# tomneda/DABstar

Hardware: AMD Instinct MI355X
Metric: DAB Mode-I ensembles/s (2.048 MS/s IQ->MSC bytes) per GPU; FIB CRC match % (higher is better)
Workload: dtype f32+i32

## Files before the change

### dabstar_amd/csrc/engine.cpp

```cpp
#include "engine.h"
#include "viterbi_core.h"
#include "fig00.h"
#include <algorithm>
#include <cstddef>
#include <cstring>
#include <map>
#include <string>
#include <tuple>
#include <vector>

int dabx_engine::build_msc_classes()
{
  const EngineDev &d = dev;
  have_fast = false;
  fast = MscFast{};
  for (void *q : fast_allocs) {
    (void)hipFree(q);
    allocs.erase(std::remove(allocs.begin(), allocs.end(), q), allocs.end());
  }
  fast_allocs.clear();
  for (auto &sc : subch_host) sc.fast_class = 0;
  if (d.max_subch <= 0) return 0;
  struct Key { int kbps, prot, shortf, cu; bool operator<(const Key &o) const { return std::tie(kbps, prot, shortf, cu) < std::tie(o.kbps, o.prot, o.shortf, o.cu); } };
  std::map<Key, std::vector<uint32_t>> groups;
// ... 674 lines not shown

int dabx_process(dabx_engine *e, int max_frames, int sync)
{
  if (!e || max_frames < 0) return DABX_E_ARG;
  if (int rc = use_device(e)) return rc;
  if (e->classes_dirty) {
    if (int rc = e->build_msc_classes()) return rc;
    e->classes_dirty = false;
  }
  if (e->dl.open && max_frames > 0) {
    const int need = (e->pending_frames + max_frames + MSC_BATCH_FRAMES - 1) / MSC_BATCH_FRAMES;
    int free_slots = 0;
    {
      std::lock_guard<std::mutex> lk(e->dl.mu);
      for (const auto &sl : e->dl.slots) free_slots += sl.state == Delivery::FREE;
    }
    if (free_slots < need) {
      set_error("dabx_process: the call closes %d chunks, %d host slabs are free (dabx_delivery_next / dabx_delivery_release)", need, free_slots);
      return DABX_E_STATE;
    }
  }
  const bool some_locked = !e->locked_host || 2 * __atomic_load_n(e->locked_host, __ATOMIC_RELAXED) >= e->dev.n_streams;
  const bool async_acquire = !e->cfg.dc_iq_correction && e->cir.n_corr == 0 && e->spectrum.n_on == 0 && (e->cfg.acquire_mode == 2 || (e->cfg.acquire_mode == 0 && some_locked));
  for (int i = 0; i < max_frames; i++) {
    if (e->ss.prep_pending && e->pending_frames >= 4) {
      DABX_HIP(hipStreamWaitEvent(e->stream, e->ss.prep_b_done, 0));
      e->ss.prep_pending = false;
    }
    const bool all_locked = e->locked_host && __atomic_load_n(e->locked_host, __ATOMIC_RELAXED) == e->dev.n_streams;
    const int cir_cap = e->cir.n_on > 0 ? cir_step_cap(e, false) : 0;
    int rc = launch_front_step(e->dev, e->ss, e->mk, async_acquire, all_locked, e->scope.n_on > 0 ? &e->scope.dev : nullptr,
                               e->cir.n_on > 0 ? &e->cir.dev : nullptr, cir_cap, e->spectrum.n_on > 0 ? &e->spectrum.dev : nullptr);
    if (rc) return rc;
    if (cir_cap > 0) cir_step_cap(e, true);
    if (e->cir.n_on > 0 && (cir_cap > 0 || e->cir.n_corr > 0)) e->cir.launches++;
    if (e->scope.n_on > 0) e->scope.launches++;
    if (e->spectrum.n_on > 0) e->spectrum.launches++;
    if (e->tiis.n_on > 0) {
      if ((rc = launch_tii(e->dev, e->tiis.dev, e->stream))) return rc;
      e->tiis.launches++;
    }
    if ((rc = fig_step(e))) return rc;
    e->level_dirty = true;
    if (++e->pending_frames == MSC_BATCH_FRAMES || i == max_frames - 1) {
      DeliverDev dv{};
      int dl_slot = -1, dl_dev = -1;
      if (e->dl.open && (rc = e->delivery_begin(&dv, &dl_slot, &dl_dev))) return rc;
      e->dev.snap = e->snap_buf[e->ss.batch_parity];
      hipStream_t tail = e->stream;
      const bool with_eti = e->dl.open && e->dl.eti();
      const EtiDev eti = with_eti ? e->dl.eti_dev(dl_dev) : EtiDev{};
      rc = launch_msc_batch(e->dev, 4 * e->pending_frames, e->have_fast ? &e->fast : nullptr, e->ss, e->mk, e->dl.open ? &dv : nullptr, &tail,
                            e->pkt.dev.n > 0 ? &e->pkt.dev : nullptr, e->pad.dev.n > 0 ? &e->pad.dev : nullptr, e->mot.dev.n > 0 ? &e->mot.dev : nullptr,
                            e->car.dev.n > 0 ? &e->car.dev : nullptr, with_eti ? &eti : nullptr, e->mpa.dev.n > 0 ? &e->mpa.dev : nullptr, &e->mpa_launches,
                            e->aac.dev.n > 0 ? &e->aac.dev : nullptr, &e->aac_launches);
      if (rc) {
// ... 412 lines not shown
```

### dabstar_amd/csrc/pipeline.h

```cpp
#pragma once
#include "dabx_internal.h"
#include "ring_fmt.h"
#include <cstddef>

namespace dabx {

#ifndef DABX_MSC_BATCH
#define DABX_MSC_BATCH 7
#endif
constexpr int MSC_SLOTS = DABX_MSC_BATCH > 7 ? 64 : 32;
constexpr int MSC_BATCH_FRAMES = DABX_MSC_BATCH;
constexpr int SF_SLOTS = 16;
constexpr int ACQ_NEED = 20 * TU + 50 + (TF + 1) + (TN + 50 + 21) + 64;
constexpr int FRAME_NEED = TF + 2 * TU;
constexpr int FEW_STREAMS = 48;

enum StreamState : int32_t { ST_INIT = 0, ST_WAIT_SYNC = 1, ST_EVAL_SYNC = 2 };

struct StreamCtl {
  unsigned long long rd;
  unsigned long long sym0_pos;
  long long cif_no;
  long long msc_done_cif;
  long long frames;
// ... 282 lines not shown
  const SubchDev &sc = e.subch[(size_t)q.s * e.max_subch + q.j];
  q.r = b.msc_done + q.k;
  const long long valid_from = sc.start_cif + 16;
  q.valid = sc.active && q.r < b.cif_no && q.r >= valid_from;
  q.out_idx = sc.cif_out + (q.r - (b.msc_done > valid_from ? b.msc_done : valid_from));
  return q;
}
__device__ __forceinline__ size_t tdi_off(long long cif, int i)
{
  return (size_t)(cif & (TDI_SLOTS - 1)) * CIF_BITS + (size_t)(i & 15) * (CIF_BITS / 16) + (size_t)(i >> 4);
}
#endif

struct PacketDev;
struct PadDev;
struct MotDev;
struct CarouselDev;
struct Mp2AudioDev;
struct AacStreamDev;
struct ScopeDev;
struct CirDev;
struct SpecDev;
extern const char *const kStepKernelNames[N_STEP_KERNELS];
int launch_front_step(const EngineDev &e, EngineStreams &ss, Marker &mk, bool async_acquire, bool all_locked, const ScopeDev *scope = nullptr,
                      const CirDev *cir = nullptr, int cir_cap = 0, const SpecDev *spec = nullptr);
int launch_msc_batch(const EngineDev &e, int cifs, const MscFast *fast, EngineStreams &ss, Marker &mk, const DeliverDev *dv = nullptr,
                     hipStream_t *tail = nullptr, const PacketDev *pk = nullptr, const PadDev *pad = nullptr, const MotDev *mot = nullptr,
                     const CarouselDev *car = nullptr, const EtiDev *eti = nullptr, const Mp2AudioDev *mp2a = nullptr, long long *mp2a_launches = nullptr,
                     const AacStreamDev *aac = nullptr, long long *aac_launches = nullptr);
int launch_dciq(const EngineDev &e, int mode, hipStream_t st);
int launch_level_exact(const EngineDev &e, hipStream_t st);
int launch_commit(const EngineDev &e, int stream, unsigned long long n, hipStream_t st);
int launch_fic_only(const EngineDev &e, hipStream_t st, int first, int count);
int launch_i16_to_sym(const int16_t *soft, uint8_t *sym, size_t n, hipStream_t st);
int launch_stage_msc_block(const EngineDev &e, const int16_t *soft_dev, int blk, bool closes_cif, hipStream_t st);
int launch_msc_inject(const EngineDev &e, int stream, const int16_t *soft_dev, int n_cifs, int first, hipStream_t st);
int launch_msc_advance(const EngineDev &e, const int32_t *counts_dev, hipStream_t st);
int launch_fic_inject(const EngineDev &e, int stream, const int16_t *soft_dev, hipStream_t st);
int launch_fic_decode(const EngineDev &e, const int32_t *present_dev, hipStream_t st);
int launch_demap_inject(const EngineDev &e, int parity, int stream, const float2 *spec_dev, const float2 *null_dev, float clock_err, int np_sel, hipStream_t st);
int launch_demap_frame(const EngineDev &e, unsigned step_count, const int32_t *present_dev, int schedule, hipStream_t st, const ScopeDev *scope = nullptr);
int launch_msc_prep(const EngineDev &e, int cifs, const MscLaunch &L, hipStream_t st, Marker &mk);
int launch_msc_vitT(const EngineDev &e, int cifs, const MscLaunch &L, hipStream_t st, Marker &mk);
int launch_deliver_front(const EngineDev &e, const DeliverDev &dv, hipStream_t st);
int launch_deliver_msc(const EngineDev &e, const DeliverDev &dv, hipStream_t st, bool with_lf);
int launch_deliver_lf(const EngineDev &e, const DeliverDev &dv, hipStream_t st);
int launch_deliver_dg(const EngineDev &e, const DeliverDev &dv, const PacketDev &pk, hipStream_t st);
int launch_deliver_pad(const EngineDev &e, const DeliverDev &dv, const PadDev &pd, hipStream_t st);
// ... 19 lines not shown
```

### dabstar_amd/csrc/pipeline.hip

```cpp
#include <type_traits>
#include "pipeline.h"
#include "packet_core.h"
#include "pad_core.h"
#include "mot_core.h"
#include "carousel_core.h"
#include "mp2_core.h"
#include "aac_core.h"
#include <algorithm>
#include "ofdm_core.h"
#include "scope_core.h"
#include "cir_core.h"
#include "spectrum_core.h"
#include "viterbi_core.h"
#include "fec_core.h"
#include "acq_walk.h"
#include "level_par.h"
#include "fig00.h"

namespace dabx {

__device__ __forceinline__ void front_prio() { __builtin_amdgcn_s_setprio(3); }

template <class T> __device__ __forceinline__ T uniform_load(const T *p)
{
// ... 583 lines not shown
    Nco nco;
    nco.init(phase0, f, tid);
    const RingView<RF> rv(ring, e.ring_len, rd);
    float2 v[8];
#pragma unroll
    for (int u = 0; u < 8; u++) { v[u] = nco.mix(rv.at(tid + 256 * u)); nco.step(); }
    const int start = prs_correlate_block(v, c.sync_thr, e.strongest, t, lds, peak, red, tid);
    __syncthreads();
    if (start >= 0) break;
    sync_failed<RF>(e, s, tid, rv, rd, phase0, f, peak, red, true);
    new_state = ST_WAIT_SYNC;
    if (wr - c.rd < (unsigned long long)(ACQ_NEED + FRAME_NEED)) break;
  }
  if (new_state < 0) return;
  if (tid == 0 && e.exact_level) e.level_pos[s] = c.rd;
  if (tid == 0 && e.anchor_level) { c.lvl_anchor_pos = c.lvl_approx_pos = c.rd; c.lvl_anchor_S = c.s_level; }
  if (tid == 0 && new_state == ST_EVAL_SYNC && e.locked_count) __hip_atomic_fetch_add(e.locked_count, 1, __ATOMIC_RELAXED, __HIP_MEMORY_SCOPE_SYSTEM);
  __threadfence();
  __syncthreads();
  if (tid == 0) __hip_atomic_store(&c.state, new_state, __ATOMIC_RELEASE, __HIP_MEMORY_SCOPE_AGENT);
}

template <int RF>
__global__ __launch_bounds__(256, RF == RING_CF32 ? 3 : 4) void k_frame_head(EngineDev e, DevTables t)
{
  front_prio();
  __shared__ float2 lds[FFT_LDS_FLOAT2];
  __shared__ __attribute__((aligned(16))) float peak[TU];
  __shared__ float red[8];
  __shared__ float mag[160];
  __shared__ int s_state;
  const int s = blockIdx.x, tid = threadIdx.x;
  StreamCtl &c = e.ctl[s];
  const typename RingFmt<RF>::Elem *ring = stream_ring<RF>(e, s);
  if (tid < 76) e.sym_off[(size_t)s * 76 + tid] = -1;
  if (tid == 0) {
    c.frame_ok = 0;
    s_state = __hip_atomic_load(&c.state, __ATOMIC_ACQUIRE, __HIP_MEMORY_SCOPE_AGENT);
  }
  __syncthreads();
  if (s_state != ST_EVAL_SYNC) return;
  __builtin_amdgcn_fence(__ATOMIC_ACQUIRE, "agent");
  if (e.wr[s] - c.rd < (unsigned long long)FRAME_NEED) return;
  const unsigned long long rd = c.rd;
  const int phase0 = c.nco_phase;
  const int f = (int)roundf(c.f_bb);
  float2 v[8];
  Nco nco;
  nco.init(phase0, f, tid);
  const RingView<RF> rv(ring, e.ring_len, rd);
  float abs_a = 0.f, abs_b = 0.f;
#pragma unroll
  for (int u = 0; u < 8; u++) { const float2 x = rv.at(tid + 256 * u); abs_a += cabsf_level(x); v[u] = nco.mix(x); nco.step(); }
  const int start = prs_correlate_block(v, c.sync_thr, e.strongest, t, lds, peak, red, tid);
// ... 34 lines not shown
    }
    if (correction != 0) clock_err = 0.0f;
    f_bb = f_sync;
  }
  e.nco_tid[(size_t)s * 256 + tid] = Nco::tid_factor((int)roundf(f_bb), tid);
  if (tid < 75) {
    double2 b, st;
    Nco::block_consts(nco_advance(phase0, f, (long long)start + TU), (int)roundf(f_bb), (long long)tid * TS + TG, b, st);
    e.nco_sym[(size_t)s * 76 + tid] = b;
    if (tid == 0) e.nco_sym[(size_t)s * 76 + 75] = st;
    e.sym_off[(size_t)s * 76 + tid] = (int32_t)((rd + (unsigned long long)start + TU + (unsigned long long)tid * TS) % (unsigned long long)e.ring_len);
  }
  if (tid == 0) {
    c.start_index = start;
    c.head_abs_a = abs_a; c.head_abs_b = abs_b;
    c.sample_count = start + TU;
    c.sym0_pos = rd + start;
    c.phase_sym1 = nco_advance(phase0, f, (long long)start + TU);
    c.correction = correction;
    c.f_sync = f_sync; c.f_bb = f_bb; c.clock_err = clock_err;
    c.f_frame = (int)roundf(f_bb);
    c.frame_ok = 1;
  }
}

__host__ __device__ constexpr int sym_blocks_per_stream(int n_streams) { return n_streams >= FEW_STREAMS ? 15 : (n_streams >= 16 ? 25 : 75); }
template <int RF>
__global__ __launch_bounds__(256, 3) void k_symbols_persistent(EngineDev e, DevTables t)
{
  front_prio();
  __shared__ float2 lds[FFT_LDS_FLOAT2];
  __shared__ float red3[3][4];
  const int s = blockIdx.y + e.s0, tid = threadIdx.x;
  int l = blockIdx.x;
  int off = uniform_load(e.sym_off + (size_t)s * 76 + l);
  double2 nco_base = uniform_load(e.nco_sym + (size_t)s * 76 + l);
  const double2 nco_step = uniform_load(e.nco_sym + (size_t)s * 76 + 75);
  if (off < 0) return;
  typedef RingFmt<RF> Fmt;
  const typename Fmt::Elem *ring = stream_ring<RF>(e, s);
  const unsigned len = (unsigned)e.ring_len;
  const bool two = tid + 256 < TG;
  typename Fmt::Elem nx[12];
  auto request = [&](int o) {
    auto at = [&](unsigned i) { unsigned a = (unsigned)o + i; if (a >= len) a -= len; return ring_elem<RF>(ring, a); };
    if (RF != RING_CF32) {
// ... 460 lines not shown

struct SrcFic {
  const uint8_t *sym;
  const uint16_t *map;
  typedef ushort4 Key;
  struct Raw { uint8_t a, b, c, d; };
  __device__ Key key(int t) const { return *reinterpret_cast<const ushort4 *>(map + 4 * t); }
  __device__ uint8_t ld(uint16_t idx) const { return sym[idx == PUNCT ? 0 : idx]; }
  __device__ Raw raw(Key m) const { return {ld(m.x), ld(m.y), ld(m.z), ld(m.w)}; }
  __device__ static int cv(uint8_t v, uint16_t idx) { return vit_sym_from_u8(idx == PUNCT ? (uint8_t)127 : v); }
  __device__ VitSyms syms(Raw r, Key m) const { return {cv(r.a, m.x), cv(r.b, m.y), cv(r.c, m.z), cv(r.d, m.w)}; }
};

__global__ __launch_bounds__(256) void k_fic_frame(EngineDev e, DevTables t, int first, int count)
{
  front_prio();
  __shared__ __attribute__((aligned(16))) char wtab[4][VIT_BLK * 16];
  __shared__ uint32_t fibw[4][24];
  __shared__ uint32_t raw[4][32];
  __shared__ uint8_t crc_ok[12];
  __shared__ uint32_t encw[4][26];
  __shared__ int ber_err[4];
  __shared__ uint16_t s_crc[256];
  const int s = blockIdx.x, wave = threadIdx.x >> 6, lane = threadIdx.x & 63;
  StreamCtl &c = e.ctl[s];
  if (e.flag_sync && first == 0 && count == 4) seq_wait(e.fic_seq + s, e.step_seq, e.seq_timeouts);
  if (!c.frame_ok) return;
  s_crc[threadIdx.x] = t.crc_ccitt[threadIdx.x];
  const int fic = first + wave;
  if (wave < count) {
    SrcFic src{e.fic_sym + (size_t)s * 3 * K2 + fic * FIC_IN, t.fic_map};
    uint32_t *dec = e.vit_scratch + ((size_t)s * 4 + fic) * (size_t)e.vit_stride;
    const VitLaneConst k = vit_lane_const(lane);
    if (e.tie_mode == 2) vit_forward<2>(src, FIC_OUT + 6, wtab[wave], dec, lane, k);
    else if (e.tie_mode) vit_forward<1>(src, FIC_OUT + 6, wtab[wave], dec, lane, k);
    else vit_forward<0>(src, FIC_OUT + 6, wtab[wave], dec, lane, k);
    __builtin_amdgcn_fence(__ATOMIC_RELEASE, "workgroup");
    __builtin_amdgcn_s_waitcnt(0);
    vit_traceback(dec, FIC_OUT, lane, raw[wave]);
    __builtin_amdgcn_fence(__ATOMIC_RELEASE, "wavefront");
    __builtin_amdgcn_wave_barrier();
    uint32_t dw = 0;
    if (lane < 24) { dw = vit_output_word(raw[wave], lane); fibw[fic][lane] = dw ^ t.prbs_words[lane]; }
    if (lane < 24) encw[wave][lane] = dw;
    if (lane >= 24 && lane < 26) encw[wave][lane] = 0;
    __builtin_amdgcn_fence(__ATOMIC_RELEASE, "wavefront");
    __builtin_amdgcn_wave_barrier();
    {
      const uint8_t *eb = reinterpret_cast<const uint8_t *>(encw[wave]);
      auto dbit = [&](int i) -> unsigned { return i < 0 ? 0u : (unsigned)((eb[i >> 3] >> (7 - (i & 7))) & 1); };
      const int t0 = 13 * lane;
      unsigned sr = 0;
#pragma unroll
      for (int q = 6; q >= 1; q--) sr = (sr << 1) | dbit(t0 - q);
      int err = 0;
      const uint8_t *sym = e.fic_sym + (size_t)s * 3 * K2 + fic * FIC_IN;
      for (int i = t0; i < t0 + 13 && i < FIC_OUT + 6; i++) {
        sr = ((sr << 1) | dbit(i)) & 0xFFu;
        const ushort4 m = *reinterpret_cast<const ushort4 *>(t.fic_map + 4 * i);
        const unsigned p0 = __builtin_popcount(sr & 109u) & 1u, p1 = __builtin_popcount(sr & 79u) & 1u, p2 = __builtin_popcount(sr & 83u) & 1u;
        if (m.x != PUNCT) err += (unsigned)(sym[m.x] > 127) != p0;
        if (m.y != PUNCT) err += (unsigned)(sym[m.y] > 127) != p1;
        if (m.z != PUNCT) err += (unsigned)(sym[m.z] > 127) != p2;
        if (m.w != PUNCT) err += (unsigned)(sym[m.w] > 127) != p0;
      }
      err = wave_sum_int(err);
      if (lane == 0) ber_err[fic] = err;
    }
  }
  __syncthreads();
  const int slot = (int)(c.frames % e.out_frames);
  uint8_t *fo = e.fib_out + ((size_t)s * e.out_frames + slot) * 12 * 32;
  const int fib0 = 3 * first, nfib = 3 * count;
  __shared__ int fib_cif[12];
  if ((int)threadIdx.x < nfib) {
    const int fibi = fib0 + threadIdx.x;
    const uint8_t *b = reinterpret_cast<const uint8_t *>(&fibw[fibi / 3][0]) + (fibi % 3) * 32;
    const uint8_t good = crc16_check_bytes(b, 30, s_crc);
    crc_ok[fibi] = good;
    e.fib_crc[((size_t)s * e.out_frames + slot) * 12 + fibi] = good;
    int cif = -1;
    int hi, lo;
    if (good && fib_fig00_counter(b, &hi, &lo)) cif = hi * 250 + lo;
    fib_cif[fibi] = cif;
  }
  for (int i = threadIdx.x; i < 24 * count; i += 256) reinterpret_cast<uint32_t *>(fo)[24 * first + i] = fibw[first + i / 24][i % 24];
  __syncthreads();
  if (threadIdx.x == 0) {
    int ratio = c.fic_ratio, cif_count = c.cif_count;
    long long ok = 0;
    for (int fibi = fib0; fibi < fib0 + nfib; fibi++) {
      if (crc_ok[fibi]) {
        ok++;
        if (fib_cif[fibi] >= 0) cif_count = fib_cif[fibi];
        if (ratio < 10) ratio++;
      } else if (ratio > 0) ratio--;
    }
    c.fic_ratio = ratio; c.cif_count = cif_count;
    c.fib_ok += ok; c.fib_total += nfib;
    int bits = c.fic_bits, errs = c.fic_errors, blk = c.fic_block;
    for (int f = first; f < first + count; f++) {
      bits += FIC_IN; errs += ber_err[f];
      if (++blk == 40) { c.fic_status_errors = errs; c.fic_status_bits = bits; blk = 0; errs /= 2; bits /= 2; }
    }
    c.fic_bits = bits; c.fic_errors = errs; c.fic_block = blk;
  }
}

template <int RF>
__global__ __launch_bounds__(256) void k_frame_tail(EngineDev e, DevTables t)
{
  front_prio();
  __shared__ float2 lds[FFT_LDS_FLOAT2];
  __shared__ float red[8];
  __shared__ float s_fbb;
  const int s = blockIdx.x, tid = threadIdx.x;
  StreamCtl &c = e.ctl[s];
  if (!c.frame_ok) return;
  const float LNQ = -1.00000500003333e-5f;
  float2 cpp = make_float2(0.f, 0.f);
  float absp = 0.f;
  if (tid < 75) { cpp = e.cp_part[(size_t)s * 75 + tid]; absp = e.abs_part[(size_t)s * 76 + tid]; }
  typedef RingFmt<RF> Fmt;
  const typename Fmt::Elem *ring = stream_ring<RF>(e, s);
  const unsigned long long base = c.sym0_pos + TU + 75ull * TS;
  const RingView<RF> rv(ring, e.ring_len, base);
  typename Fmt::Elem xr[8];
#pragma unroll
  for (int u = 0; u < 8; u++) xr[u] = rv.code(TG + tid + 256 * u);
  constexpr int N_REST = (TN - TU + 255) / 256;
  typename Fmt::Elem xq[N_REST];
#pragma unroll
  for (int k = 0; k < N_REST; k++) {
    const int i = min(tid + 256 * k, TN - TU - 1);
    xq[k] = rv.code(i < TG ? i : i + TU);
  }
  asm volatile("" ::: "memory");
  float cre = cpp.x, cim = cpp.y, sym_w = 0.f;
// ... 65 lines not shown
      auto upd = [&lv](float mean, float qn) { lv += (1.0f - qn) * (mean - lv); };
      const int start = c.start_index;
      upd(c.head_abs_a * (1.0f / (float)TU), __expf((float)TU * LNQ));
      if (start > 0) upd(c.head_abs_b / (float)start, __expf((float)start * LNQ));
      lv = lv * __expf((float)(75 * TS) * LNQ) + (1.0f - __expf((float)TS * LNQ)) * sym_w;
      upd(an * (1.0f / (float)TN), __expf((float)TN * LNQ));
      if (!e.exact_level) c.s_level = lv;
    }
    if (e.frame_pos) {
      const size_t slot = (size_t)s * e.out_frames + (size_t)(c.frames % e.out_frames);
      e.frame_pos[slot] = (long long)c.sym0_pos; e.frame_start[slot] = c.start_index;
    }
    c.sample_count = sample_count;
    c.rd = base + TN;
    c.lvl_approx_pos = c.rd;
    { const int h = (int)(c.frames % LVL_HIST); c.lvl_hist_pos[h] = c.rd; c.lvl_hist_S[h] = c.s_level; }
    c.nco_phase = nco_advance(phase_null, f2, TN);
    c.cif_no += 4;
    c.frames += 1;
    c.np_sel ^= 1;
    c.sync_thr = 2.0f * e.threshold;
    c.state = ST_EVAL_SYNC;
  }
}

template <int RF>
__global__ __launch_bounds__(128) void k_level_exact(EngineDev e)
{
  front_prio();
  const int s = blockIdx.x, tid = threadIdx.x, lane = tid & 63;
  const int wave = __builtin_amdgcn_readfirstlane(tid >> 6);
  StreamCtl &c = e.ctl[s];
  constexpr int CH = 1024;
  __shared__ __attribute__((aligned(16))) float chunk[2][CH + 32];
  const unsigned long long rd0 = e.level_pos[s];
  const unsigned long long rd1 = __hip_atomic_load(&c.rd, __ATOMIC_RELAXED, __HIP_MEMORY_SCOPE_AGENT);
  if (rd1 <= rd0) return;
  const unsigned long long n = rd1 - rd0;
  typedef RingFmt<RF> Fmt;
  const typename Fmt::Elem *ring = stream_ring<RF>(e, s);
  const unsigned len = (unsigned)e.ring_len;
  typename Fmt::Elem raw[CH / 64];
  unsigned raw_ok = 0;
  __shared__ float s_pk;
  auto request = [&](unsigned long long p0) {
    const unsigned o0 = (unsigned)((rd0 + p0) % len);
// ... 445 lines not shown
}

int launch_spectrum_rows_test(const float2 *in, int n, float *state, float *lin, float *db, float *ext, const float *window, hipStream_t st)
{
  const DevTables *t;
  if (int rc = get_tables(&t)) return rc;
  hipLaunchKernelGGL(k_spectrum_rows_test, dim3(1), dim3(256), 0, st, in, n, state, lin, db, ext, window, *t);
  DABX_HIP(hipGetLastError());
  return 0;
}

static int launch_spectrum(const EngineDev &e, const DevTables &t, const SpecDev *sd, hipStream_t st)
{
  if (!sd || sd->n <= 0) return 0;
  DABX_LAUNCH_RING(e, k_spectrum, dim3(sd->n), dim3(256), 0, st, e, t, *sd);
  DABX_HIP(hipGetLastError());
  return 0;
}

const char *const kStepKernelNames[N_STEP_KERNELS] = {"k_acquire", "k_frame_head", "k_symbols", "k_demap_frame", "k_fic_frame", "k_frame_tail",
                                                      "k_msc_prep", "k_msc_vitT", "k_msc_frame", "k_dabplus", "k_demap_fic", "k_packet", "k_pad", "k_mot",
                                                      "k_carousel", "k_eti"};

int launch_front_step(const EngineDev &e_in, EngineStreams &ss, Marker &mk, bool async_acquire, bool all_locked, const ScopeDev *scope, const CirDev *cir, int cir_cap,
                      const SpecDev *spec)
{
  const DevTables *t;
  int rc = get_tables(&t);
  if (rc) return rc;
  EngineDev e = e_in;
  e.parity = (int)(ss.step_count++ & 1u);
  e.step_seq = ss.step_count;
  e.flag_sync = (ss.d && ss.fic_on_d && e.sym_seq) ? 1 : 0;
  hipStream_t st = ss.a;
  if (all_locked && !e.exact_level) {
  } else if (async_acquire && ss.q) {
    const bool go = !ss.acq_in_flight || hipEventQuery(ss.acq_done) == hipSuccess;
    if (go || e.exact_level) {
      if (ss.acq_a_pending) { DABX_HIP(hipStreamWaitEvent(ss.q, ss.acq_a_done, 0)); ss.acq_a_pending = false; }
      if (e.exact_level) {
        if (ss.tail_recorded) DABX_HIP(hipStreamWaitEvent(ss.q, ss.tail_done, 0));
        DABX_LAUNCH_RING(e, k_level_exact, dim3(e.n_streams), dim3(128), 0, ss.q, e);
      }
      if (go) { mk.begin(0, ss.q); DABX_LAUNCH_RING(e, k_acquire, dim3(e.n_streams), dim3(256), 0, ss.q, e, *t, 1); mk.end(0, ss.q); }
      DABX_HIP(hipEventRecord(ss.acq_done, ss.q));
      ss.acq_in_flight = true;
    }
  } else {
    if (ss.acq_in_flight) { DABX_HIP(hipStreamWaitEvent(st, ss.acq_done, 0)); ss.acq_in_flight = false; }
    if (e.exact_level) DABX_LAUNCH_RING(e, k_level_exact, dim3(e.n_streams), dim3(128), 0, st, e);
    mk.begin(0, st); DABX_LAUNCH_RING(e, k_acquire, dim3(e.n_streams), dim3(256), 0, st, e, *t, 1); mk.end(0, st);
    if (ss.q && ss.acq_a_done) { DABX_HIP(hipEventRecord(ss.acq_a_done, st)); ss.acq_a_pending = true; }
  }
  if ((rc = launch_cir(e, *t, cir, cir_cap, st))) return rc;
  if ((rc = launch_cir_corr(e, *t, cir, st))) return rc;
  mk.begin(1, st); DABX_LAUNCH_RING(e, k_frame_head, dim3(e.n_streams), dim3(256), 0, st, e, *t); mk.end(1, st);
  if ((rc = launch_spectrum(e, *t, spec, st))) return rc;
  mk.begin(2, st); DABX_LAUNCH_RING(e, k_symbols_persistent, dim3(sym_blocks_per_stream(e.n_streams), e.n_streams), dim3(256), 0, st, e, *t); mk.end(2, st);
#define DABX_DEMAP_DISPATCH(KERNEL, ...)                                                                                         \
  do {                                                                                                                          \
    const int st_ = e.demap.soft_type == 3 ? 3 : e.demap.soft_type == 2 ? 2 : 1;                                                \
    if (e.demap.track_mer) {                                    \
      if (e.tie_mode) {                                                                                                         \
        if (st_ == 3) hipLaunchKernelGGL((KERNEL<3, true, true>), __VA_ARGS__);                                                 \
        else if (st_ == 2) hipLaunchKernelGGL((KERNEL<2, true, true>), __VA_ARGS__);                                            \
        else hipLaunchKernelGGL((KERNEL<1, true, true>), __VA_ARGS__);                                                          \
      } else {                                                                                                                  \
        if (st_ == 3) hipLaunchKernelGGL((KERNEL<3, false, true>), __VA_ARGS__);                                                \
        else if (st_ == 2) hipLaunchKernelGGL((KERNEL<2, false, true>), __VA_ARGS__);                                           \
        else hipLaunchKernelGGL((KERNEL<1, false, true>), __VA_ARGS__);                                                         \
      }                                                                                                                         \
    } else if (e.tie_mode) {                                                                                                    \
      if (st_ == 3) hipLaunchKernelGGL((KERNEL<3, true, false>), __VA_ARGS__);                                                  \
      else if (st_ == 2) hipLaunchKernelGGL((KERNEL<2, true, false>), __VA_ARGS__);                                             \
      else hipLaunchKernelGGL((KERNEL<1, true, false>), __VA_ARGS__);                                                           \
    } else {                                                                                                                    \
      if (st_ == 3) hipLaunchKernelGGL((KERNEL<3, false, false>), __VA_ARGS__);                                                 \
      else if (st_ == 2) hipLaunchKernelGGL((KERNEL<2, false, false>), __VA_ARGS__);                                            \
      else hipLaunchKernelGGL((KERNEL<1, false, false>), __VA_ARGS__);                                                          \
// ... 5 lines not shown
  if (ss.d && ss.fic_on_d) {
    hipLaunchKernelGGL(k_sym_publish, dim3((e.n_streams + 63) / 64), dim3(64), 0, st, e);
    if ((rc = launch_scope(e, *t, scope, ss.d))) return rc;
    mk.begin(3, ss.d);
    DABX_DEMAP_DISPATCH(k_demap_whole, dim3(e.n_streams), dim3(DEMAP_THREADS), 0, ss.d, e, *t);
    mk.end(3, ss.d);
    ss.demap_in_flight = true; ss.demap_unrecorded = true;
  } else if (ss.d) {
    if (ss.demap_in_flight) { DABX_HIP(hipStreamWaitEvent(st, ss.demap_done, 0)); ss.demap_in_flight = false; }
    if ((rc = launch_scope(e, *t, scope, st))) return rc;
    mk.begin(10, st);
    DABX_DEMAP_DISPATCH(k_demap_fic, dim3(e.n_streams), dim3(DEMAP_THREADS), 0, st, e, *t);
    mk.end(10, st);
    DABX_HIP(hipEventRecord(ss.fic_go, st));
    DABX_HIP(hipStreamWaitEvent(ss.d, ss.fic_go, 0));
    mk.begin(3, ss.d); demap(ss.d, 3, 75); mk.end(3, ss.d);
    DABX_HIP(hipEventRecord(ss.demap_done, ss.d));
    ss.demap_in_flight = true;
  } else {
    if ((rc = launch_scope(e, *t, scope, st))) return rc;
    mk.begin(3, st); demap(st, 0, 75); mk.end(3, st);
  }
  mk.begin(4, st); hipLaunchKernelGGL(k_fic_frame, dim3(e.n_streams), dim3(256), 0, st, e, *t, 0, 4); mk.end(4, st);
  mk.begin(5, st); DABX_LAUNCH_RING(e, k_frame_tail, dim3(e.n_streams), dim3(256), 0, st, e, *t); mk.end(5, st);
  if (e.exact_level && ss.tail_done) { DABX_HIP(hipEventRecord(ss.tail_done, st)); ss.tail_recorded = true; }
  DABX_HIP(hipGetLastError());
  return 0;
}

int launch_msc_batch(const EngineDev &e, int cifs, const MscFast *fast, EngineStreams &ss, Marker &mk, const DeliverDev *dv, hipStream_t *tail,
                     const PacketDev *pk, const PadDev *pad, const MotDev *mot, const CarouselDev *car, const EtiDev *eti, const Mp2AudioDev *mp2a,
                     long long *mp2a_launches, const AacStreamDev *aac, long long *aac_launches)
{
  const DevTables *t;
  int rc = get_tables(&t);
  if (rc) return rc;
  if (tail) *tail = ss.a;
  if (e.fic_only || e.max_subch <= 0 || !e.msc_out) {
    if (dv && (rc = launch_deliver_msc(e, *dv, ss.a, true))) return rc;
    if (dv && eti && (rc = launch_eti_back(e, *eti, ss.a, mk, false))) return rc;
    return 0;
  }
  const int jobs = e.n_streams * cifs * e.max_subch;
  auto wait_for_demapper = [&](hipStream_t who) -> int {
    if (!ss.demap_in_flight) return 0;
    if (ss.demap_unrecorded) { DABX_HIP(hipEventRecord(ss.demap_done, ss.d)); ss.demap_unrecorded = false; }
    DABX_HIP(hipStreamWaitEvent(who, ss.demap_done, 0));
// ... 253 lines not shown
```

### dabstar_amd/csrc/viterbi_core.h

```cpp
#pragma once
#include <hip/hip_runtime.h>
#include <stdint.h>
#include "wave_ops.h"

namespace dabx {

constexpr int VIT_BLK = 60;
constexpr int VIT_DW = 30;

__host__ __device__ inline int vit_words(int nbits) { return (nbits + 6 + VIT_DW - 1) / VIT_DW; }
__host__ __device__ inline int vit_blocks(int nbits) { return (nbits + 6 + VIT_BLK - 1) / VIT_BLK; }
__host__ __device__ inline size_t vit_scratch_words(int nbits) { return (size_t)vit_blocks(nbits) * 2 * 64; }

struct VitSyms { int x0, x1, x2, x3; };

__device__ __forceinline__ int vit_sym_from_i16(int16_t s)
{
  int v = (int16_t)(s + 127);
  v = v < 0 ? 0 : (v > 255 ? 255 : v);
  return 2 * v - 255;
}
__device__ __forceinline__ int vit_sym_from_u8(uint8_t sym) { return 2 * (int)sym - 255; }
__device__ __forceinline__ int vit_sym_from_i16_sat(int16_t s)
{
  int v = (int)s + 127;
// ... 79 lines not shown
__device__ __forceinline__ void vit_step_simd(int &m, unsigned &acc, const char *wrow, const VitLaneConst &k)
{
  constexpr int CEIL = RULE == 1 ? 65535 : 32767;
  const int w = *reinterpret_cast<const int16_t *>(wrow + k.pat[C]);
  const int bm = (w + 1020) >> 1;
  const int partner = vit_exchange<C>(m, k.lane);
  int a = m + bm, b = partner + (1020 - bm);
  a = a > CEIL ? CEIL : a; b = b > CEIL ? CEIL : b;
  const int dd = __mul24(a - b, k.sgn[C]);
  m = a < b ? a : b;
  if constexpr (RULE == 1) asm("v_cmp_le_i32 vcc, 0, %1\n\tv_addc_co_u32 %0, vcc, %0, %0, vcc" : "+v"(acc) : "v"(dd) : "vcc");
  else asm("v_cmp_lt_i32 vcc, 0, %1\n\tv_addc_co_u32 %0, vcc, %0, %0, vcc" : "+v"(acc) : "v"(dd) : "vcc");
}
__device__ __forceinline__ int vit_wave_min(int v) { return wave_min_int(v); }
template <int C, int RULE>
__device__ __forceinline__ void vit_pair_simd(int &m, unsigned &acc, const char *row, const VitLaneConst &k)
{
  vit_step_simd<C, RULE>(m, acc, row, k);
  const int m0_before = __builtin_amdgcn_readfirstlane(m);
  vit_step_simd<C + 1, RULE>(m, acc, row + 16, k);
  if (m0_before > (RULE == 1 ? 60000 : 30000)) m -= vit_wave_min(m);
}

template <int RULE = 0, class Src>
__device__ __forceinline__ void vit_forward(const Src &src, int nsteps, char *wtab, uint32_t *dec, int lane,
                                            const VitLaneConst &k)
{
  int m = RULE ? (lane == 0 ? 0 : 1000) : (lane == 0 ? 0 : 2000);
  const int nblk = (nsteps + VIT_BLK - 1) / VIT_BLK;
  const bool fetcher = lane < VIT_BLK;
  auto tclamp = [&](int t) { return t < nsteps ? t : 0; };
  typename Src::Key k1 = src.key(tclamp(lane));
  typename Src::Raw rw = src.raw(k1);
  VitSyms s = src.syms(rw, k1);
  if (!(fetcher && lane < nsteps)) s = VitSyms{0, 0, 0, 0};
  k1 = src.key(tclamp(VIT_BLK + lane));
  for (int b = 0; b < nblk; b++) {
    const int tn = (b + 1) * VIT_BLK + lane;
    const typename Src::Raw rn = src.raw(k1);
    const typename Src::Key kn = k1;
    k1 = src.key(tclamp(tn + VIT_BLK));
    if (lane < VIT_BLK) {
      const int y0 = s.x0 + s.x3;
      short v[8];
#pragma unroll
      for (int q = 0; q < 8; q++)
        v[q] = (short)(((q & 4) ? -y0 : y0) + ((q & 2) ? -s.x1 : s.x1) + ((q & 1) ? -s.x2 : s.x2));
      int4 pk;
      pk.x = (unsigned short)v[0] | ((unsigned)(unsigned short)v[1] << 16);
      pk.y = (unsigned short)v[2] | ((unsigned)(unsigned short)v[3] << 16);
      pk.z = (unsigned short)v[4] | ((unsigned)(unsigned short)v[5] << 16);
      pk.w = (unsigned short)v[6] | ((unsigned)(unsigned short)v[7] << 16);
      *reinterpret_cast<int4 *>(wtab + lane * 16) = pk;
    }
    __builtin_amdgcn_fence(__ATOMIC_RELEASE, "wavefront");
    __builtin_amdgcn_wave_barrier();
    unsigned acc = 0;
#pragma unroll
    for (int h = 0; h < VIT_BLK / VIT_DW; h++) {
#pragma unroll
      for (int s6 = 0; s6 < VIT_DW; s6 += 6) {
        const char *row = wtab + (h * VIT_DW + s6) * 16;
        if constexpr (RULE != 0) {
          vit_pair_simd<0, RULE>(m, acc, row + 0 * 16, k);
          vit_pair_simd<2, RULE>(m, acc, row + 2 * 16, k);
          vit_pair_simd<4, RULE>(m, acc, row + 4 * 16, k);
        } else {
          vit_step<0>(m, acc, row + 0 * 16, k);
          vit_step<1>(m, acc, row + 1 * 16, k);
          vit_step<2>(m, acc, row + 2 * 16, k);
          vit_step<3>(m, acc, row + 3 * 16, k);
          vit_step<4>(m, acc, row + 4 * 16, k);
          vit_step<5>(m, acc, row + 5 * 16, k);
        }
      }
      dec[(size_t)(b * (VIT_BLK / VIT_DW) + h) * 64 + lane] = RULE == 0 ? acc ^ k.inv30 : acc;
      acc = 0;
    }
    __builtin_amdgcn_wave_barrier();
    s = src.syms(rn, kn);
    if (!(fetcher && tn < nsteps)) s = VitSyms{0, 0, 0, 0};
  }
}

constexpr int VIT_RAW_WORDS = 312;

struct VitMask6 { unsigned long long m5, m4, m3, m2, m1, m0; };
template <int G> __device__ __forceinline__ VitMask6 vit_tb_masks(unsigned hist)
{
  VitMask6 r;
  r.m5 = __builtin_amdgcn_ballot_w64(((hist >> (VIT_DW - 1 - (6 * G + 5))) & 1u) != 0u);
  r.m4 = __builtin_amdgcn_ballot_w64(((hist >> (VIT_DW - 1 - (6 * G + 4))) & 1u) != 0u);
  r.m3 = __builtin_amdgcn_ballot_w64(((hist >> (VIT_DW - 1 - (6 * G + 3))) & 1u) != 0u);
  r.m2 = __builtin_amdgcn_ballot_w64(((hist >> (VIT_DW - 1 - (6 * G + 2))) & 1u) != 0u);
  r.m1 = __builtin_amdgcn_ballot_w64(((hist >> (VIT_DW - 1 - (6 * G + 1))) & 1u) != 0u);
  r.m0 = __builtin_amdgcn_ballot_w64(((hist >> (VIT_DW - 1 - (6 * G + 0))) & 1u) != 0u);
  return r;
}
__device__ __forceinline__ void vit_tb_chain(const VitMask6 &q, int &j, unsigned &acc)
{
  int jc, js;
#define DABX_TB_STEP(M, BIT)                                                                                                    \
  "s_andn2_b32 %[jc], %[j], " #BIT "\n\ts_or_b32 %[js], %[j], " #BIT "\n\ts_bitcmp1_b64 %[" #M "], %[j]\n\t"                        \
  "s_cselect_b32 %[j], %[js], %[jc]\n\t"
  asm volatile(DABX_TB_STEP(m5, 1) DABX_TB_STEP(m4, 2) DABX_TB_STEP(m3, 4) DABX_TB_STEP(m2, 8) DABX_TB_STEP(m1, 16) DABX_TB_STEP(m0, 32)
               "s_brev_b32 %[jc], %[j]\n\ts_lshl_b32 %[acc], %[acc], 6\n\ts_lshr_b32 %[jc], %[jc], 26\n\ts_or_b32 %[acc], %[acc], %[jc]"
               : [jc] "=&s"(jc), [js] "=&s"(js), [acc] "+s"(acc), [j] "+s"(j)
               : [m5] "s"(q.m5), [m4] "s"(q.m4), [m3] "s"(q.m3), [m2] "s"(q.m2), [m1] "s"(q.m1), [m0] "s"(q.m0)
               : "scc");
#undef DABX_TB_STEP
}
template <int NG>
__device__ __forceinline__ VitMask6 vit_tb_word(unsigned hist, unsigned nxt, VitMask6 ahead, int &j, unsigned &acc)
{
  VitMask6 a = ahead;
  if constexpr (NG >= 5) { const VitMask6 b = vit_tb_masks<3>(hist); vit_tb_chain(a, j, acc); a = b; }
  if constexpr (NG >= 4) { const VitMask6 b = vit_tb_masks<2>(hist); vit_tb_chain(a, j, acc); a = b; }
  if constexpr (NG >= 3) { const VitMask6 b = vit_tb_masks<1>(hist); vit_tb_chain(a, j, acc); a = b; }
  if constexpr (NG >= 2) { const VitMask6 b = vit_tb_masks<0>(hist); vit_tb_chain(a, j, acc); a = b; }
  const VitMask6 b = vit_tb_masks<4>(nxt);
  vit_tb_chain(a, j, acc);
  return b;
}

__device__ __forceinline__ void vit_traceback(const uint32_t *dec, int nbits, int lane, uint32_t *raw)
{
  const int nsteps = __builtin_amdgcn_readfirstlane(nbits + 6);
  int j = 0;
  int wi = (nsteps - 1) / VIT_DW;
  unsigned hist = dec[(size_t)wi * 64 + lane];
  VitMask6 ahead;
  {
    const unsigned nxt = wi > 0 ? dec[(size_t)(wi - 1) * 64 + lane] : 0u;
    unsigned acc = 0;
    const int n_top = nsteps - wi * VIT_DW;
    if (n_top % 6 == 0) {
      switch (n_top / 6) {
        case 5: ahead = vit_tb_word<5>(hist, nxt, vit_tb_masks<4>(hist), j, acc); break;
        case 4: ahead = vit_tb_word<4>(hist, nxt, vit_tb_masks<3>(hist), j, acc); break;
        case 3: ahead = vit_tb_word<3>(hist, nxt, vit_tb_masks<2>(hist), j, acc); break;
        case 2: ahead = vit_tb_word<2>(hist, nxt, vit_tb_masks<1>(hist), j, acc); break;
        default: ahead = vit_tb_word<1>(hist, nxt, vit_tb_masks<0>(hist), j, acc); break;
      }
    } else {
      for (int s = n_top - 1; s >= 0; --s) {
        const unsigned hv = (unsigned)__builtin_amdgcn_readlane((int)hist, __builtin_amdgcn_readfirstlane(j));
        const unsigned k = (hv >> (VIT_DW - 1 - s)) & 1u;
        acc = (acc << 1) | k;
// ... 32 lines not shown
```

Measured before the change: 564,900.

## Fuse frame tail with next frame head and keep FIC Viterbi decisions in LDS

Adds a k_frame_turn kernel that runs the current frame's tail and the next frame's head in one launch. The host loop uses it when no intervening launches (CIR, spectrum, TII, FIG, exact level) are needed and the next frame is known to be locked or acquired asynchronously, which saves one kernel launch and one grid-wide dependency per frame. Separately, the FIC Viterbi path now writes decision words to LDS instead of global scratch, and it records hard bits and puncture flags during the forward pass so the BER re-encode no longer re-reads symbols and the map from global memory. The risks are higher LDS use in k_fic_frame, lower occupancy, and the head decision depending on host-side lock state that was read one frame early.

```diff
diff --git a/dabstar_amd/csrc/engine.cpp b/dabstar_amd/csrc/engine.cpp
--- a/dabstar_amd/csrc/engine.cpp
+++ b/dabstar_amd/csrc/engine.cpp
@@ -720,16 +720,26 @@
   }
   const bool some_locked = !e->locked_host || 2 * __atomic_load_n(e->locked_host, __ATOMIC_RELAXED) >= e->dev.n_streams;
   const bool async_acquire = !e->cfg.dc_iq_correction && e->cir.n_corr == 0 && e->spectrum.n_on == 0 && (e->cfg.acquire_mode == 2 || (e->cfg.acquire_mode == 0 && some_locked));
+  const auto locked_now = [&] { return e->locked_host && __atomic_load_n(e->locked_host, __ATOMIC_RELAXED) == e->dev.n_streams; };
+  const bool turn_ok = !e->dev.exact_level && e->cir.n_on == 0 && e->spectrum.n_on == 0 && e->tiis.n_on == 0 && e->fig.n_on == 0;
+  bool head_done = false, all_locked = false;
   for (int i = 0; i < max_frames; i++) {
     if (e->ss.prep_pending && e->pending_frames >= 4) {
       DABX_HIP(hipStreamWaitEvent(e->stream, e->ss.prep_b_done, 0));
       e->ss.prep_pending = false;
     }
-    const bool all_locked = e->locked_host && __atomic_load_n(e->locked_host, __ATOMIC_RELAXED) == e->dev.n_streams;
+    if (!head_done) all_locked = locked_now();
+    bool turn = false, next_locked = false;
+    if (turn_ok && i + 1 < max_frames && e->pending_frames + 1 < MSC_BATCH_FRAMES) {
+      next_locked = locked_now();
+      turn = next_locked || (async_acquire && e->ss.q);
+    }
     const int cir_cap = e->cir.n_on > 0 ? cir_step_cap(e, false) : 0;
-    int rc = launch_front_step(e->dev, e->ss, e->mk, async_acquire, all_locked, e->scope.n_on > 0 ? &e->scope.dev : nullptr,
+    int rc = launch_front_step(e->dev, e->ss, e->mk, async_acquire, all_locked, head_done, turn, e->scope.n_on > 0 ? &e->scope.dev : nullptr,
                                e->cir.n_on > 0 ? &e->cir.dev : nullptr, cir_cap, e->spectrum.n_on > 0 ? &e->spectrum.dev : nullptr);
     if (rc) return rc;
+    head_done = turn;
+    all_locked = next_locked;
     if (cir_cap > 0) cir_step_cap(e, true);
     if (e->cir.n_on > 0 && (cir_cap > 0 || e->cir.n_corr > 0)) e->cir.launches++;
     if (e->scope.n_on > 0) e->scope.launches++;
diff --git a/dabstar_amd/csrc/pipeline.h b/dabstar_amd/csrc/pipeline.h
--- a/dabstar_amd/csrc/pipeline.h
+++ b/dabstar_amd/csrc/pipeline.h
@@ -328,8 +328,8 @@
 struct CirDev;
 struct SpecDev;
 extern const char *const kStepKernelNames[N_STEP_KERNELS];
-int launch_front_step(const EngineDev &e, EngineStreams &ss, Marker &mk, bool async_acquire, bool all_locked, const ScopeDev *scope = nullptr,
-                      const CirDev *cir = nullptr, int cir_cap = 0, const SpecDev *spec = nullptr);
+int launch_front_step(const EngineDev &e, EngineStreams &ss, Marker &mk, bool async_acquire, bool all_locked, bool head_done, bool turn,
+                      const ScopeDev *scope = nullptr, const CirDev *cir = nullptr, int cir_cap = 0, const SpecDev *spec = nullptr);
 int launch_msc_batch(const EngineDev &e, int cifs, const MscFast *fast, EngineStreams &ss, Marker &mk, const DeliverDev *dv = nullptr,
                      hipStream_t *tail = nullptr, const PacketDev *pk = nullptr, const PadDev *pad = nullptr, const MotDev *mot = nullptr,
                      const CarouselDev *car = nullptr, const EtiDev *eti = nullptr, const Mp2AudioDev *mp2a = nullptr, long long *mp2a_launches = nullptr,
diff --git a/dabstar_amd/csrc/pipeline.hip b/dabstar_amd/csrc/pipeline.hip
--- a/dabstar_amd/csrc/pipeline.hip
+++ b/dabstar_amd/csrc/pipeline.hip
@@ -629,14 +629,8 @@
 }
 
 template <int RF>
-__global__ __launch_bounds__(256, RF == RING_CF32 ? 3 : 4) void k_frame_head(EngineDev e, DevTables t)
-{
-  front_prio();
-  __shared__ float2 lds[FFT_LDS_FLOAT2];
-  __shared__ __attribute__((aligned(16))) float peak[TU];
-  __shared__ float red[8];
-  __shared__ float mag[160];
-  __shared__ int s_state;
+__device__ __forceinline__ void frame_head_body(EngineDev &e, const DevTables &t, float2 *lds, float *peak, float *red, float *mag, int &s_state)
+{
   const int s = blockIdx.x, tid = threadIdx.x;
   StreamCtl &c = e.ctl[s];
   const typename RingFmt<RF>::Elem *ring = stream_ring<RF>(e, s);
@@ -717,6 +711,18 @@
     c.f_frame = (int)roundf(f_bb);
     c.frame_ok = 1;
   }
+}
+
+template <int RF>
+__global__ __launch_bounds__(256, RF == RING_CF32 ? 3 : 4) void k_frame_head(EngineDev e, DevTables t)
+{
+  front_prio();
+  __shared__ float2 lds[FFT_LDS_FLOAT2];
+  __shared__ __attribute__((aligned(16))) float peak[TU];
+  __shared__ float red[8];
+  __shared__ float mag[160];
+  __shared__ int s_state;
+  frame_head_body<RF>(e, t, lds, peak, red, mag, s_state);
 }
 
 __host__ __device__ constexpr int sym_blocks_per_stream(int n_streams) { return n_streams >= FEW_STREAMS ? 15 : (n_streams >= 16 ? 25 : 75); }
@@ -1223,6 +1229,9 @@
   __shared__ uint32_t encw[4][26];
   __shared__ int ber_err[4];
   __shared__ uint16_t s_crc[256];
+  constexpr int FIC_DEC_WORDS = (FIC_OUT + 6 + VIT_BLK - 1) / VIT_BLK * (VIT_BLK / VIT_DW);
+  __shared__ uint32_t decw[4][FIC_DEC_WORDS * 64];
+  __shared__ uint8_t hard[4][(FIC_OUT + 6 + 15) / 16 * 16];
   const int s = blockIdx.x, wave = threadIdx.x >> 6, lane = threadIdx.x & 63;
   StreamCtl &c = e.ctl[s];
   if (e.flag_sync && first == 0 && count == 4) seq_wait(e.fic_seq + s, e.step_seq, e.seq_timeouts);
@@ -1231,13 +1240,18 @@
   const int fic = first + wave;
   if (wave < count) {
     SrcFic src{e.fic_sym + (size_t)s * 3 * K2 + fic * FIC_IN, t.fic_map};
-    uint32_t *dec = e.vit_scratch + ((size_t)s * 4 + fic) * (size_t)e.vit_stride;
+    VitLdsWord *dec = (VitLdsWord *)decw[wave];
+    uint8_t *hd = hard[wave];
+    const auto note = [hd](int tt, const SrcFic::Raw &r, const SrcFic::Key &m) {
+      hd[tt] = (uint8_t)((unsigned)(r.a > 127) | ((unsigned)(r.b > 127) << 1) | ((unsigned)(r.c > 127) << 2) | ((unsigned)(r.d > 127) << 3) |
+                         ((unsigned)(m.x != PUNCT) << 4) | ((unsigned)(m.y != PUNCT) << 5) | ((unsigned)(m.z != PUNCT) << 6) | ((unsigned)(m.w != PUNCT) << 7));
+    };
     const VitLaneConst k = vit_lane_const(lane);
-    if (e.tie_mode == 2) vit_forward<2>(src, FIC_OUT + 6, wtab[wave], dec, lane, k);
-    else if (e.tie_mode) vit_forward<1>(src, FIC_OUT + 6, wtab[wave], dec, lane, k);
-    else vit_forward<0>(src, FIC_OUT + 6, wtab[wave], dec, lane, k);
-    __builtin_amdgcn_fence(__ATOMIC_RELEASE, "workgroup");
-    __builtin_amdgcn_s_waitcnt(0);
+    if (e.tie_mode == 2) vit_forward<2>(src, FIC_OUT + 6, wtab[wave], dec, lane, k, note);
+    else if (e.tie_mode) vit_forward<1>(src, FIC_OUT + 6, wtab[wave], dec, lane, k, note);
+    else vit_forward<0>(src, FIC_OUT + 6, wtab[wave], dec, lane, k, note);
+    __builtin_amdgcn_fence(__ATOMIC_RELEASE, "wavefront");
+    __builtin_amdgcn_wave_barrier();
     vit_traceback(dec, FIC_OUT, lane, raw[wave]);
     __builtin_amdgcn_fence(__ATOMIC_RELEASE, "wavefront");
     __builtin_amdgcn_wave_barrier();
@@ -1255,15 +1269,14 @@
 #pragma unroll
       for (int q = 6; q >= 1; q--) sr = (sr << 1) | dbit(t0 - q);
       int err = 0;
-      const uint8_t *sym = e.fic_sym + (size_t)s * 3 * K2 + fic * FIC_IN;
       for (int i = t0; i < t0 + 13 && i < FIC_OUT + 6; i++) {
         sr = ((sr << 1) | dbit(i)) & 0xFFu;
-        const ushort4 m = *reinterpret_cast<const ushort4 *>(t.fic_map + 4 * i);
+        const unsigned h = hd[i];
         const unsigned p0 = __builtin_popcount(sr & 109u) & 1u, p1 = __builtin_popcount(sr & 79u) & 1u, p2 = __builtin_popcount(sr & 83u) & 1u;
-        if (m.x != PUNCT) err += (unsigned)(sym[m.x] > 127) != p0;
-        if (m.y != PUNCT) err += (unsigned)(sym[m.y] > 127) != p1;
-        if (m.z != PUNCT) err += (unsigned)(sym[m.z] > 127) != p2;
-        if (m.w != PUNCT) err += (unsigned)(sym[m.w] > 127) != p0;
+        if (h & 16u) err += (h & 1u) != p0;
+        if (h & 32u) err += ((h >> 1) & 1u) != p1;
+        if (h & 64u) err += ((h >> 2) & 1u) != p2;
+        if (h & 128u) err += ((h >> 3) & 1u) != p0;
       }
       err = wave_sum_int(err);
       if (lane == 0) ber_err[fic] = err;
@@ -1309,12 +1322,8 @@
 }
 
 template <int RF>
-__global__ __launch_bounds__(256) void k_frame_tail(EngineDev e, DevTables t)
-{
-  front_prio();
-  __shared__ float2 lds[FFT_LDS_FLOAT2];
-  __shared__ float red[8];
-  __shared__ float s_fbb;
+__device__ __forceinline__ void frame_tail_body(EngineDev &e, const DevTables &t, float2 *lds, float *red, float &s_fbb)
+{
   const int s = blockIdx.x, tid = threadIdx.x;
   StreamCtl &c = e.ctl[s];
   if (!c.frame_ok) return;
@@ -1426,6 +1435,31 @@
     c.sync_thr = 2.0f * e.threshold;
     c.state = ST_EVAL_SYNC;
   }
+}
+
+template <int RF>
+__global__ __launch_bounds__(256) void k_frame_tail(EngineDev e, DevTables t)
+{
+  front_prio();
+  __shared__ float2 lds[FFT_LDS_FLOAT2];
+  __shared__ float red[8];
+  __shared__ float s_fbb;
+  frame_tail_body<RF>(e, t, lds, red, s_fbb);
+}
+
+template <int RF>
+__global__ __launch_bounds__(256, 4) void k_frame_turn(EngineDev e, DevTables t)
+{
+  front_prio();
+  __shared__ float2 lds[FFT_LDS_FLOAT2];
+  __shared__ __attribute__((aligned(16))) float peak[TU];
+  __shared__ float red[8];
+  __shared__ float mag[160];
+  __shared__ int s_state;
+  __shared__ float s_fbb;
+  frame_tail_body<RF>(e, t, lds, red, s_fbb);
+  __syncthreads();
+  frame_head_body<RF>(e, t, lds, peak, red, mag, s_state);
 }
 
 template <int RF>
@@ -1917,9 +1951,13 @@
                                                       "k_msc_prep", "k_msc_vitT", "k_msc_frame", "k_dabplus", "k_demap_fic", "k_packet", "k_pad", "k_mot",
                                                       "k_carousel", "k_eti"};
 
-int launch_front_step(const EngineDev &e_in, EngineStreams &ss, Marker &mk, bool async_acquire, bool all_locked, const ScopeDev *scope, const CirDev *cir, int cir_cap,
-                      const SpecDev *spec)
-{
+int launch_front_step(const EngineDev &e_in, EngineStreams &ss, Marker &mk, bool async_acquire, bool all_locked, bool head_done, bool turn,
+                      const ScopeDev *scope, const CirDev *cir, int cir_cap, const SpecDev *spec)
+{
+  if (((head_done || turn) && (e_in.exact_level || cir || spec)) || (head_done && !(all_locked || (async_acquire && ss.q)))) {
+    set_error("launch_front_step: a frame turn with a launch between tail and head");
+    return DABX_E_ARG;
+  }
   const DevTables *t;
   int rc = get_tables(&t);
   if (rc) return rc;
@@ -1949,7 +1987,7 @@
   }
   if ((rc = launch_cir(e, *t, cir, cir_cap, st))) return rc;
   if ((rc = launch_cir_corr(e, *t, cir, st))) return rc;
-  mk.begin(1, st); DABX_LAUNCH_RING(e, k_frame_head, dim3(e.n_streams), dim3(256), 0, st, e, *t); mk.end(1, st);
+  if (!head_done) { mk.begin(1, st); DABX_LAUNCH_RING(e, k_frame_head, dim3(e.n_streams), dim3(256), 0, st, e, *t); mk.end(1, st); }
   if ((rc = launch_spectrum(e, *t, spec, st))) return rc;
   mk.begin(2, st); DABX_LAUNCH_RING(e, k_symbols_persistent, dim3(sym_blocks_per_stream(e.n_streams), e.n_streams), dim3(256), 0, st, e, *t); mk.end(2, st);
 #define DABX_DEMAP_DISPATCH(KERNEL, ...)                                                                                         \
@@ -2001,7 +2039,10 @@
     mk.begin(3, st); demap(st, 0, 75); mk.end(3, st);
   }
   mk.begin(4, st); hipLaunchKernelGGL(k_fic_frame, dim3(e.n_streams), dim3(256), 0, st, e, *t, 0, 4); mk.end(4, st);
-  mk.begin(5, st); DABX_LAUNCH_RING(e, k_frame_tail, dim3(e.n_streams), dim3(256), 0, st, e, *t); mk.end(5, st);
+  mk.begin(5, st);
+  if (turn) DABX_LAUNCH_RING(e, k_frame_turn, dim3(e.n_streams), dim3(256), 0, st, e, *t);
+  else DABX_LAUNCH_RING(e, k_frame_tail, dim3(e.n_streams), dim3(256), 0, st, e, *t);
+  mk.end(5, st);
   if (e.exact_level && ss.tail_done) { DABX_HIP(hipEventRecord(ss.tail_done, st)); ss.tail_recorded = true; }
   DABX_HIP(hipGetLastError());
   return 0;
diff --git a/dabstar_amd/csrc/viterbi_core.h b/dabstar_amd/csrc/viterbi_core.h
--- a/dabstar_amd/csrc/viterbi_core.h
+++ b/dabstar_amd/csrc/viterbi_core.h
@@ -1,6 +1,7 @@
 #pragma once
 #include <hip/hip_runtime.h>
 #include <stdint.h>
+#include <type_traits>
 #include "wave_ops.h"
 
 namespace dabx {
@@ -126,9 +127,11 @@
   if (m0_before > (RULE == 1 ? 60000 : 30000)) m -= vit_wave_min(m);
 }
 
-template <int RULE = 0, class Src>
-__device__ __forceinline__ void vit_forward(const Src &src, int nsteps, char *wtab, uint32_t *dec, int lane,
-                                            const VitLaneConst &k)
+typedef __attribute__((address_space(3))) uint32_t VitLdsWord;
+struct VitNoNote { template <class R, class K> __device__ __forceinline__ void operator()(int, const R &, const K &) const {} };
+template <int RULE = 0, class Src, class Dec, class Note = VitNoNote>
+__device__ __forceinline__ void vit_forward(const Src &src, int nsteps, char *wtab, Dec dec, int lane,
+                                            const VitLaneConst &k, const Note &note = Note())
 {
   int m = RULE ? (lane == 0 ? 0 : 1000) : (lane == 0 ? 0 : 2000);
   const int nblk = (nsteps + VIT_BLK - 1) / VIT_BLK;
@@ -138,6 +141,7 @@
   typename Src::Raw rw = src.raw(k1);
   VitSyms s = src.syms(rw, k1);
   if (!(fetcher && lane < nsteps)) s = VitSyms{0, 0, 0, 0};
+  else note(lane, rw, k1);
   k1 = src.key(tclamp(VIT_BLK + lane));
   for (int b = 0; b < nblk; b++) {
     const int tn = (b + 1) * VIT_BLK + lane;
@@ -179,11 +183,13 @@
         }
       }
       dec[(size_t)(b * (VIT_BLK / VIT_DW) + h) * 64 + lane] = RULE == 0 ? acc ^ k.inv30 : acc;
+      if constexpr (std::is_same<Dec, VitLdsWord *>::value) __builtin_amdgcn_sched_barrier(0);
       acc = 0;
     }
     __builtin_amdgcn_wave_barrier();
     s = src.syms(rn, kn);
     if (!(fetcher && tn < nsteps)) s = VitSyms{0, 0, 0, 0};
+    else note(tn, rn, kn);
   }
 }
 
@@ -227,7 +233,8 @@
   return b;
 }
 
-__device__ __forceinline__ void vit_traceback(const uint32_t *dec, int nbits, int lane, uint32_t *raw)
+template <class Dec>
+__device__ __forceinline__ void vit_traceback(Dec dec, int nbits, int lane, uint32_t *raw)
 {
   const int nsteps = __builtin_amdgcn_readfirstlane(nbits + 6);
   int j = 0;
```

New measurement: 565,500, median of 2. About the same (+0.1%).
